# ThinkLib/Sail

Measured on AMD Instinct MI355X. Metric: Msamples/s (paths x bounces) at 1920x1080 Cornell box, higher is better.
Workload: dtype f32; 1 GPU; cornell_box_readme_C2; width=1920, height=1080, bounces=8, spp=1024, launch_spp=1024, partition=tiles64x1, processes=one

## Files before the change

sail_amd/capi.py:

```python
from __future__ import annotations

import ctypes
import os
from typing import Optional, Sequence

import numpy as np

_HERE = os.path.dirname(os.path.abspath(__file__))
LIB_PATH = os.environ.get("SAIL_HIP_LIB") or os.path.join(_HERE, "lib", "libsail_hip.so")

SAIL_OK = 0
FLAG_AOV = 1
FLAG_SEGMENT_COUNT = 2
ACCUM_SUM, ACCUM_MIX, ACCUM_COMPAT8 = 0, 1, 2
PART_TILES, PART_SAMPLES = 0, 1
FILTER_COLOR, FILTER_GAMMA, FILTER_TONEMAPPING, FILTER_WINDOW = 0, 1, 2, 3
FILTER_WAVELET, FILTER_NORMAL, FILTER_POSITION = 4, 5, 6
DEBUG_CULL_MIN_PRIMS, DEBUG_FORCE_GENERIC, DEBUG_CULL_FMA, DEBUG_SAMPLE_GROUPS, DEBUG_FORCE_RCCL = 1, 2, 3, 4, 5
DEBUG_WAVEFRONT = 6
DEBUG_GROUP_ROUNDS = 7
DEBUG_CULL_GROUP_ROUNDS = 8
DEBUG_JIT = 9
DEBUG_JIT_WAIT = 10
DEBUG_JIT_NT = 12
DEBUG_JIT_NS = 11
DEBUG_JIT_VALUES_AFTER = 13
KERNEL_JIT_NONE, KERNEL_JIT_PENDING, KERNEL_JIT_READY, KERNEL_JIT_FAILED = 0, 1, 2, 3
JIT_MODE_FLAT, JIT_MODE_CULL, JIT_MODE_ROOM = 0, 1, 2
DEBUG_DEFAULTS: dict = {}

EXPORTS = (
    "sail_create", "sail_create_multi", "sail_set_debug", "sail_destroy", "sail_last_error", "sail_device_count", "sail_device_info", "sail_set_scene",
    "sail_update_objects", "sail_set_accum_mode", "sail_set_partition", "sail_set_launch_samples",
    "sail_render", "sail_render_schedule", "sail_reset", "sail_sync", "sail_readback", "sail_read_accum",
    "sail_filter", "sail_get_stats", "sail_camera", "sail_jitter_inverse", "sail_schedule",
    "sail_comm_unique_id", "sail_comm_init", "sail_reduce", "sail_accum_device_ptr", "sail_partition_tiles",
    "sail_prim_bounds", "sail_math_probe", "sail_pick", "sail_kernel_name", "sail_filter_ms",
    "sail_abi_version", "sail_accum_parts", "sail_save_accum", "sail_load_accum", "sail_jit_compile",
    "sail_get_kernel_info", "sail_kernel_ready", "sail_set_jit_cache", "sail_jit_prebuild",
    "sail_jit_value_key", "sail_jit_spec_key", "sail_plan_settle", "sail_jit_resident",
    "sail_plan_reduce", "sail_plan_keep", "sail_plan_load_part", "sail_plan_last_bounce",
    "sail_noise_mark", "sail_noise_estimate", "sail_plan_until", "sail_render_until",
    "sail_set_active_tiles", "sail_get_active_tiles", "sail_plan_adaptive", "sail_adaptive_defaults", "sail_render_adaptive",
    "sail_denoise_defaults", "sail_denoise",
    "sail_temporal_defaults", "sail_gbuffer", "sail_temporal_begin", "sail_temporal_resolve", "sail_temporal_read",
    "sail_temporal_load_history",
    "sail_temporal_moments", "sail_temporal_load_moments", "sail_temporal_read_moments",
    "sail_temporal_filter_defaults", "sail_temporal_filter",
    "sail_move_objects", "sail_temporal_pending_motion",
    "sail_albedo", "sail_albedo_load", "sail_albedo_read", "sail_denoise_albedo", "sail_temporal_filter_albedo",
)


class SailError(RuntimeError):
    pass
# ... 970 lines not shown
```

sail_amd/csrc/sail_capi.cpp:

```cpp
#include <hip/hip_runtime.h>
#include <dlfcn.h>
#include <math.h>
#include <algorithm>
#include <cmath>
#include <stdarg.h>
#include <stdio.h>
#include <stdlib.h>
#include <string.h>
#include <string>
#include <vector>
#include "sail_ctx.h"

namespace {

thread_local std::string g_create_error;

float gdiv(float a, float b) { return a * (1.0f / b); }

int texel(float c, int size) {
  if (c != c) return 0;
  const float s = floorf(c * (float)size);
  if (!(s >= 0.0f)) return 0;
  if (s >= (float)(size - 1)) return size - 1;
  return (int)s;
// ... 154 lines not shown
          for (int k = 0; k < 3; k++) {
            volatile float f = kd * sc[q][k];
            f = f * kInvPI;
            if (!std::isfinite((float)f)) matteOk = false;
          }
      }
    }
    if (emPosZero && matteOk) *quietRows |= 1u << i;
    else if (!(matteOk && !emBlack)) skip = false;
  }
  *skipSort = (any && skip) ? 1 : 0;
}
bool valueSpecFor(const SailJitSpec& types, const std::vector<uint32_t>& rowWords, const float* tp, int tn, int jit, SailJitSpec* out) {
  const bool cornellSet = (types.ks & ~SAIL_KSET_CORNELL_SHAPES) == 0 && (types.km & ~SAIL_KSET_CORNELL_MATS) == 0 &&
                          (types.kt & ~SAIL_KSET_CORNELL_TEX) == 0 && types.kl == 0;
  if (!cornellSet || types.mode != SAIL_JIT_MODE_FLAT || types.rows <= 0 || types.tn != 0 || tn < 0 || tn > kSailJitMaxFlatTp ||
      rowWords.size() != (size_t)types.rows * 32 || (tn > 0 && !tp))
    return false;
  *out = types;
  out->rowWords = rowWords;
  out->tpWords.resize((size_t)tn * 16);
  if (tn > 0) memcpy(out->tpWords.data(), tp, sizeof(float) * 16 * (size_t)tn);
  out->rowForm = out->rowShade = out->rowQuiet = 0;
  if ((jit & 32) && types.rows <= kSailJitRowRecordMax) {
    out->rowForm = 1;
    std::vector<SailPrim> prims((size_t)types.rows);
    memcpy(prims.data(), rowWords.data(), sizeof(SailPrim) * prims.size());
    uint32_t quiet = 0;
    int skip = 0;
    lastBounceRows(prims, tp, tn, types.km, false, &quiet, &skip);
    out->rowShade = (int)(quiet & ((1u << types.rows) - 1u));
    out->rowQuiet = out->rowShade;
  }
  return true;
}
void refreshValues(sail_ctx* c) {
  if (!c->subs.empty() || c->valueSlot.have || !c->typesSlot.have || !settledFor(c->settled, c->jitValuesAfter)) return;
  SailJitSpec spec;
  if (!valueSpecFor(c->typesSlot.spec, c->rowWords, c->tpRows.data(), c->tn, c->jit, &spec)) return;
  c->valueSlot.adopt(c->device, c->stream, spec);
}
void refreshJit(sail_ctx* c) {
  if (!c->subs.empty()) return;
  SailJitSpec spec;
  int mode = 0;
  const bool have = jitSpecFor(c, &spec, &mode);
  if (have == c->typesSlot.have && (!have || sailJitSpecEqual(spec, c->typesSlot.spec))) return;
  dropValues(c);
  c->typesTwin.drop(c->device, c->stream);
  if (have) c->typesSlot.adopt(c->device, c->stream, spec);
  else c->typesSlot.drop(c->device, c->stream);
}
JitSlot* maskedTwin(sail_ctx* c, JitSlot& twin, const JitSlot& base) {
  SailJitSpec want = base.spec;
  want.masked = 1;
  if (!twin.have || !sailJitSpecEqual(twin.spec, want)) twin.adopt(c->device, c->stream, want);
  return twin.poll(c->device, c->jitWait) ? &twin : nullptr;
}
JitSlot* runningSlot(sail_ctx* c, bool masked, bool wavefront) {
  if (wavefront) return nullptr;
  if (c->valueSlot.poll(c->device, 0)) {
    JitSlot* s = masked ? maskedTwin(c, c->valueTwin, c->valueSlot) : &c->valueSlot;
    if (s) return s;
  }
  if (c->typesSlot.poll(c->device, c->jitWait)) return masked ? maskedTwin(c, c->typesTwin, c->typesSlot) : &c->typesSlot;
  return nullptr;
// ... 657 lines not shown
  if (!c) return SAIL_E_INVALID;
  if (option == SAIL_DEBUG_FORCE_RCCL) {
    if (c->subs.empty() || c->groupLocal)
      return fail(c, SAIL_E_INVALID, "SAIL_DEBUG_FORCE_RCCL needs a multi-device context of distinct devices");
    for (sail_ctx* s : c->subs) if (int rc = flushQueued(s)) return relay(c, rc, s);
    const int nd = (int)c->subs.size();
    if (value && c->groupComms.empty()) {
      if (!g_rccl.load()) return fail(c, SAIL_E_RCCL, "librccl not loadable");
      std::vector<int> dev((size_t)nd);
      for (int i = 0; i < nd; i++) dev[i] = c->subs[i]->device;
      c->groupComms.assign((size_t)nd, nullptr);
      const int r = g_rccl.commInitAll(c->groupComms.data(), nd, dev.data());
      if (r) {
        c->groupComms.clear();
        return fail(c, SAIL_E_RCCL, "ncclCommInitAll: %s", g_rccl.errStr ? g_rccl.errStr(r) : "?");
      }
    } else if (!value && nd == 1 && !c->groupComms.empty()) {
      for (sail_ctx* s : c->subs) { (void)hipSetDevice(s->device); (void)hipStreamSynchronize(s->stream); }
      for (nccl_comm_t cm : c->groupComms) if (cm) g_rccl.commDestroy(cm);
      c->groupComms.clear();
    }
    c->dirty = true;
    return SAIL_OK;
  }
  for (sail_ctx* s : c->subs) if (int rc = sail_set_debug(s, option, value)) return relay(c, rc, s);
  if (int rc = flushQueued(c)) return rc;
  switch (option) {
    case SAIL_DEBUG_CULL_MIN_PRIMS: c->cullMinPrims = value; break;
    case SAIL_DEBUG_FORCE_GENERIC: c->forceGeneric = value; break;
    case SAIL_DEBUG_CULL_FMA: c->cullFma = value; break;
    case SAIL_DEBUG_SAMPLE_GROUPS: c->forceGroups = value; break;
    case SAIL_DEBUG_WAVEFRONT: c->wavefront = value; break;
    case SAIL_DEBUG_JIT:
      if ((c->jit ^ value) & 32) { const uint64_t s = c->settled; dropValues(c); c->settled = s; }
      c->jit = value;
      break;
    case SAIL_DEBUG_JIT_NT:
      if (value != 0 && value != 128 && value != 256 && value != 512 && value != 1024)
        return fail(c, SAIL_E_INVALID, "sail_set_debug: threads per workgroup must be 0 (default), 128, 256, 512 or 1024");
      c->jitNt = value;
      break;
    case SAIL_DEBUG_JIT_NS:
      if (value != 0 && value != 1 && value != 4 && value != 16)
        return fail(c, SAIL_E_INVALID, "sail_set_debug: samples in flight must be 0 (default), 1, 4 or 16");
      c->jitNs = value;
      break;
    case SAIL_DEBUG_JIT_WAIT:
      if (value < -1) return fail(c, SAIL_E_INVALID, "sail_set_debug: jit wait must be >= -1");
      c->jitWait = value;
      break;
    case SAIL_DEBUG_JIT_VALUES_AFTER:
      c->jitValuesAfter = value;
      if (value < 0) { const uint64_t s = c->settled; dropValues(c); c->settled = s; }
      break;
    case SAIL_DEBUG_GROUP_ROUNDS:
      if (value <= 0) return fail(c, SAIL_E_INVALID, "sail_set_debug: group rounds must be > 0");
      c->flatGroupRounds = value;
      break;
    case SAIL_DEBUG_CULL_GROUP_ROUNDS:
      if (value <= 0) return fail(c, SAIL_E_INVALID, "sail_set_debug: group rounds must be > 0");
      c->cullGroupRounds = value;
      break;
    default: return fail(c, SAIL_E_INVALID, "sail_set_debug: unknown option %d", option);
  }
  refreshJit(c);
  refreshValues(c);
  return SAIL_OK;
// ... 614 lines not shown
```

sail_amd/csrc/sail_geom.h:

```cpp
#pragma once
#if !defined(__HIPCC_RTC__)
#include <hip/hip_runtime.h>
#include <stdint.h>
#endif
#include "sail_device.h"
#include "sail_math.h"

using namespace sm;

#define D __device__ __forceinline__

namespace {

constexpr float kMaxDistance = 1e5f, kEps = 1e-5f, kOneMinusEps = 0.9999f, kInf = 1e5f;
constexpr float kPI = 3.141592653589793f, kInvPI = 0.3183098861837907f;
constexpr float kPiOver2 = 1.570796326794896f, kPiOver4 = 0.785398163397448f;

struct V3 { float x, y, z; };
struct V2 { float x, y; };
D V3 v3(float x, float y, float z) { V3 r; r.x = x; r.y = y; r.z = z; return r; }
D V3 v3s(float s) { return v3(s, s, s); }
D V2 v2(float x, float y) { V2 r; r.x = x; r.y = y; return r; }
D V3 operator+(V3 a, V3 b) { return v3(a.x + b.x, a.y + b.y, a.z + b.z); }
D V3 operator-(V3 a, V3 b) { return v3(a.x - b.x, a.y - b.y, a.z - b.z); }
// ... 13 lines not shown
D V3 vmin(V3 a, V3 b) { return v3(fmin_(a.x, b.x), fmin_(a.y, b.y), fmin_(a.z, b.z)); }
D V3 vmax(V3 a, V3 b) { return v3(fmax_(a.x, b.x), fmax_(a.y, b.y), fmax_(a.z, b.z)); }
D V3 vclamp01(V3 x) { return v3(clamp_(x.x, 0.0f, 1.0f), clamp_(x.y, 0.0f, 1.0f), clamp_(x.z, 0.0f, 1.0f)); }
D bool isBlack(V3 a) { return a.x == 0.0f && a.y == 0.0f && a.z == 0.0f; }
D V3 reflect_(V3 I, V3 N) { return I - (2.0f * dot(N, I)) * N; }
D V3 refract_(V3 I, V3 N, float eta) {
  const float dni = dot(N, I);
  const float k = 1.0f - eta * eta * (1.0f - dni * dni);
  if (k < 0.0f) return v3s(0.0f);
  return eta * I - (eta * dni + sqrtf_(k)) * N;
}
D V3 worldToLocal(V3 v, V3 ns, V3 ss, V3 ts) { return v3(dot(v, ss), dot(v, ts), dot(v, ns)); }
D V3 localToWorld(V3 v, V3 ns, V3 ss, V3 ts) {
  return v3(ss.x * v.x + ts.x * v.y + ns.x * v.z, ss.y * v.x + ts.y * v.y + ns.y * v.z,
            ss.z * v.x + ts.z * v.y + ns.z * v.z);
}
D float dotX(V3 a, V3 b) { return fma_(a.z, b.z, fma_(a.y, b.y, a.x * b.x)); }
D V3 crossX(V3 a, V3 b) {
  return v3(fma_(a.y, b.z, -(a.z * b.y)), fma_(a.z, b.x, -(a.x * b.z)), fma_(a.x, b.y, -(a.y * b.x)));
}
D V3 localToWorldX(V3 v, V3 ns, V3 ss, V3 ts) {
  return v3(fma_(ns.x, v.z, fma_(ts.x, v.y, ss.x * v.x)), fma_(ns.y, v.z, fma_(ts.y, v.y, ss.y * v.x)),
            fma_(ns.z, v.z, fma_(ts.z, v.y, ss.z * v.x)));
}
D V3 W2L(V3 v) {
  return v3(fma_(v.y, 0.0f, v.x * 0.0f) - v.z, fma_(v.z, 0.0f, fma_(v.y, 0.0f, v.x)), fma_(v.z, 0.0f, fma_(v.x, 0.0f, v.y)));
}
D V3 L2W(V3 v) {
  return v3(fma_(v.z, 0.0f, fma_(v.x, 0.0f, v.y)), fma_(v.y, 0.0f, v.x * 0.0f) + v.z, fma_(v.z, 0.0f, fma_(v.y, 0.0f, -v.x)));
}
D bool equalZero(float x) { return x < 1e-3f && x > -1e-3f; }
D float sgn(int rev) { return rev ? -1.0f : 1.0f; }

D bool quadratic(float A, float B, float C, float& t0, float& t1) {
  const float discrim = B * B - 4.0f * A * C;
  if (discrim < 0.0f) return false;
  const float rootDiscrim = sqrtf_(discrim);
  float q;
  if (B < 0.0f) q = -0.5f * (B - rootDiscrim);
  else q = -0.5f * (B + rootDiscrim);
  t0 = fdiv(q, A);
  t1 = fdiv(C, q);
  if (t0 > t1) { const float tmp = t0; t0 = t1; t1 = tmp; }
  return true;
}

struct Ray { V3 o, d; float rx, ry, rz; };
D Ray mkRay(V3 o, V3 d) {
  Ray r; r.o = o; r.d = d;
  const float mx = fmaxf(fmaxf(fabsf(d.x), fabsf(d.y)), fabsf(d.z)), mn = fminf(fminf(fabsf(d.x), fabsf(d.y)), fabsf(d.z));
  if (__builtin_expect(__builtin_amdgcn_ballot_w64(!(mn >= 0x1p-126f && mx <= 0x1p126f)) == 0ull, 1)) {
    const float y0 = __builtin_amdgcn_rcpf(d.x), y1 = __builtin_amdgcn_rcpf(d.y), y2 = __builtin_amdgcn_rcpf(d.z);
    r.rx = fma_(fma_(-d.x, y0, 1.0f), y0, y0);
    r.ry = fma_(fma_(-d.y, y1, 1.0f), y1, y1);
    r.rz = fma_(fma_(-d.z, y2, 1.0f), y2, y2);
  } else {
    r.rx = 1.0f / d.x; r.ry = 1.0f / d.y; r.rz = 1.0f / d.z;
  }
  return r;
}
struct Hit {
  float d; V3 hit, normal, dpdu, dpdv; bool into; int matRow; V3 sc, emission; int matCategory;
  float nd;
  bool axis;
};
struct Ctx {
  const float* tp; const float* lt; const int32_t* lightObjRow; const SailPrim* prims;
  const SailPrim* cprims;
  const float* tpl;
  bool rowCopy, tpCopy;
  const unsigned long long* typeMasks;
  int n, tn, ln;
  uint32_t matMask, texMask, lightMask;
  float fcx, fcy;
  int shadowAnyHit;
  int cullPrims;
  int cullFma;
  int cullPrimary;
  uint32_t kShapes, kMats, kTex, kLights;
};
#define HAS(set, id) (((set) >> (id)) & 1u)

template <typename T> using ConstAS = const __attribute__((address_space(4))) T;
template <typename T> D const T& constRow(const T* base, int i) { return *(const T*)((ConstAS<T>*)base + i); }
#if defined(SAIL_JIT) && defined(SAIL_JIT_ROWVALS) && SAIL_JIT_ROWVALS && SAIL_JIT_N > 0
#define SAIL_ROWVALS 1
template <class... T> constexpr int wordCount(T...) { return (int)sizeof...(T); }
static_assert(sizeof(SailPrim) == 128, "a row is 32 words");
static_assert(wordCount(SAIL_JIT_ROW_WORDS) == SAIL_JIT_N * 32, "32 words per row");
constexpr int kTpC = SAIL_JIT_TPN;
static_assert(wordCount(SAIL_JIT_TP_WORDS) == (kTpC > 0 ? kTpC * 16 : 1), "16 words per texParams row");
struct PrimWordsC { uint32_t w[SAIL_JIT_N * 32]; };
struct PrimTabC { SailPrim r[SAIL_JIT_N]; };
struct TpWordsC { uint32_t w[kTpC > 0 ? kTpC * 16 : 1]; };
struct TpTabC { float v[kTpC > 0 ? kTpC * 16 : 1]; };
constexpr PrimWordsC kPrimW = {{SAIL_JIT_ROW_WORDS}};
constexpr TpWordsC kTpW = {{SAIL_JIT_TP_WORDS}};
constexpr PrimTabC kPrimTab = __builtin_bit_cast(PrimTabC, kPrimW);
constexpr TpTabC kTpTab = __builtin_bit_cast(TpTabC, kTpW);
#define PRIM(c, i) (kPrimTab.r[(i)])
#else
#define SAIL_ROWVALS 0
#define PRIM(c, i) constRow<SailPrim>((c).prims, (i))
#endif
#if SAIL_ROWVALS && defined(SAIL_JIT_ROWSHADE) && SAIL_JIT_ROWSHADE
#define SAIL_ROWSHADE 1
#else
#define SAIL_ROWSHADE 0
#endif

D V3 P3(const SailPrim& p, int k) { return v3(p.a[k], p.a[k + 1], p.a[k + 2]); }
D float TP(const Ctx& c, int row, int col) {
#if SAIL_ROWVALS
  return kTpTab.v[row * 16 + col];
#else
  if (c.tpCopy) return c.tpl[row * 16 + col];
  return constRow<float>(c.tp, row * 16 + col);
#endif
}
D V3 TP3(const Ctx& c, int row, int col) { return v3(TP(c, row, col), TP(c, row, col + 1), TP(c, row, col + 2)); }

D int matCat(const SailPrim& p) { return (int)(short)(p.cats & 0xffff); }
D int texCat(const SailPrim& p) { return p.cats >> 16; }
D bool needsUV(const SailPrim& p) { return texCat(p) != SAIL_TEX_UNIFORM; }
D V3 getSurfaceColor(const Ctx& c, V2 uv, const SailPrim& p) {
  const int texRow = p.texRow, cat = texCat(p);
  if (cat == SAIL_TEX_UNIFORM) return TP3(c, texRow, 1);
  if (cat < 0 || cat >= 32 || !((c.texMask >> cat) & 1u)) return v3s(0.0f);
  if (c.cullPrims &&
      ((cat == SAIL_TEX_CHECKERBOARD && HAS(c.kTex, SAIL_TEX_CHECKERBOARD)) ||
       (cat == SAIL_TEX_CHECKERBOARD2 && HAS(c.kTex, SAIL_TEX_CHECKERBOARD2)))) {
    const bool cb1 = cat == SAIL_TEX_CHECKERBOARD;
    const float size = cb1 ? TP(c, texRow, 1) : TP(c, texRow, 7);
    const float sx = fdiv(uv.x, size), sy = fdiv(uv.y, size);
    const float qx = floorf(sx), qy = floorf(sy);
    if (cb1) {
      const float width = fdiv(0.5f * TP(c, texRow, 2), size);
      const float fx = sx - qx, fy = sy - qy;
      const bool in_outline = (fx < width || fx > 1.0f - width) || (fy < width || fy > 1.0f - width);
      return in_outline ? v3s(0.5f) : v3s(1.0f);
    }
    return (to_int(qx + qy) % 2 == 0) ? TP3(c, texRow, 1) : TP3(c, texRow, 4);
// ... 103 lines not shown
  if (x.x < mn.x + 0.0001f) h.sc = v3(0.25f, 0.75f, 0.25f);
  else if (x.x > mx.x - 0.0001f) h.sc = v3(0.25f, 0.25f, 0.75f);
  else if (x.y < mn.y + 0.0001f) h.sc = v3s(1.0f);
  else if (x.y > mx.y - 0.0001f) h.sc = v3s(1.0f);
  else if (x.z > mn.z + 0.0001f) h.sc = v3s(1.0f);
  else h.sc = v3s(0.0f);
}

D void boxHit(const Ctx& c, const SailPrim& p, const Ray& r, float t, Hit& h, bool cornell) {
  h.hit = r.o + t * r.d;
  const float s = cornell ? -1.0f : sgn(p.rev);
  h.normal = s * normalForCornellbox(r.o + t * r.d, p);
  dpdBox(h.normal, h.dpdu, h.dpdv);
  const V3 mn = P3(p, 0), mx = P3(p, 3), x = h.hit;
  if (cornell) {
    if (x.x < mn.x + 0.0001f) h.sc = v3(0.25f, 0.75f, 0.25f);
    else if (x.x > mx.x - 0.0001f) h.sc = v3(0.25f, 0.25f, 0.75f);
    else if (x.y < mn.y + 0.0001f) h.sc = v3s(1.0f);
    else if (x.y > mx.y - 0.0001f) h.sc = v3s(1.0f);
    else if (x.z > mn.z + 0.0001f) h.sc = v3s(1.0f);
    else h.sc = v3s(0.0f);
  } else {
    V2 uv = v2(0.0f, 0.0f);
    if (needsUV(p)) {
      const V3 tr = mx - mn, hh = h.hit - mn;
      if (hh.x < mn.x + 0.0001f || hh.x > mx.x - 0.0001f) uv = v2(fdiv(hh.y, tr.y), fdiv(hh.z, tr.z));
      else if (hh.y < mn.y + 0.0001f || hh.y > mx.y - 0.0001f) uv = v2(fdiv(hh.x, tr.x), fdiv(hh.z, tr.z));
      else uv = v2(fdiv(hh.x, tr.x), fdiv(hh.y, tr.y));
    }
    h.sc = getSurfaceColor(c, uv, p);
  }
}

D float sphereT(const SailPrim& p, const Ray& r0, V3* hitOut) {
  const V3 c = P3(p, 0);
  const float rad = p.a[3];
  const V3 d = W2L(r0.d), o = W2L(r0.o - c);
  const float a = dot(d, d), b = 2.0f * dot(o, d), cc = dot(o, o) - rad * rad;
  float t1 = 0.0f, t2 = 0.0f;
  if (!quadratic(a, b, cc, t1, t2)) return kMaxDistance;
  if (t2 < kEps) return kMaxDistance;
  float t = t1;
  if (t1 < kEps) t = t2;
  if (t >= kMaxDistance) return kMaxDistance;
  if (!testBoundbox(r0, c - v3s(rad), c + v3s(rad))) return kMaxDistance;
  if (hitOut) *hitOut = o + t * d;
  return t;
}
D float phiOf(float y, float x) {
  float phi = atan2f_(y, x);
  if (phi < 0.0f) phi += 2.0f * kPI;
  return phi;
}
D V3 dpduRot(V3 hit) { return v3(-2.0f * kPI * hit.y, 2.0f * kPI * hit.x, 0.0f); }
D V3 crossZa(V3 a, V3 b) {
  return v3(fma_(b.y, -0.0f, a.y * b.z), fma_(b.x, 0.0f, -(a.x * b.z)), a.x * b.y - a.y * b.x);
}
D V3 crossZb(V3 a, V3 b) {
  return v3(fma_(a.y, 0.0f, -(a.z * b.y)), fma_(a.x, -0.0f, a.z * b.x), a.x * b.y - a.y * b.x);
}
D void sphereHit(const Ctx& c, const SailPrim& p, V3 hl, Hit& h) {
  const float rad = p.a[3];
  const float theta = acosf_(clamp_(fdiv(hl.z, rad), -1.0f, 1.0f));
  V2 uv = v2(0.0f, 0.0f);
  if (needsUV(p)) {
    V3 hit = hl;
    if (hit.x == 0.0f && hit.y == 0.0f) hit.x = 1e-5f * rad;
    uv = v2(fdiv(phiOf(hit.y, hit.x), 2.0f * kPI), fdiv(theta, kPI));
  }
  const float th2 = theta;
  const float zRadius = sqrtf_(hl.x * hl.x + hl.y * hl.y);
  const float invZRadius = rcp_rn(zRadius);
  const float cosPhi = hl.x * invZRadius, sinPhi = hl.y * invZRadius;
  const V3 dpdu = dpduRot(hl);
  const V3 dpdv = kPI * v3(hl.z * cosPhi, hl.z * sinPhi, -rad * sinf_(th2));
  const V3 nl = normalize(crossZb(dpdv, dpdu));
  h.sc = getSurfaceColor(c, uv, p);
  h.hit = L2W(hl) + P3(p, 0);
  h.normal = L2W(nl);
  h.dpdu = L2W(dpdu);
// ... 514 lines not shown
      best = t;
      if (c.shadowAnyHit && best > kEps && best < kOneMinusEps) break;
    }
  }
  return best;
}

struct Sweep { float best; int bi; V3 bhl; };
D Sweep sweepRay(const Ctx& c, const Ray& r, bool primary) {
  float best = kMaxDistance;
  int bi = -1;
  V3 bhl = v3s(0.0f);
  const bool cull = c.cullPrims && (!primary || c.cullPrimary);
  if (cull) {
    candSweep<true>(c, r, kMaxDistance, best, bi, bhl);
    Sweep sw; sw.best = best; sw.bi = bi; sw.bhl = bhl;
    return sw;
  }
  if constexpr (kRows > 0) {
    if (!c.cullPrims) {
      sweepRows<0>(c, r, best, bi, bhl);
      Sweep sw; sw.best = best; sw.bi = bi; sw.bhl = bhl;
      return sw;
    }
  }
  for (int i = 0; i < c.n; i++) {
    V3 hl = v3s(0.0f);
    const float t = primT(c, PRIM(c, i), r, &hl);
    if (t < best) { best = t; bi = i; bhl = hl; }
  }
  Sweep sw; sw.best = best; sw.bi = bi; sw.bhl = bhl;
  return sw;
}
D V3 quadLocalHit(const SailPrim& p, const Ray& r, float t) {
  const V3 d = W2L(r.d), o = W2L(r.o - P3(p, 0));
  return o + t * d;
}
D V3 rectLocalHit(const SailPrim& p, const Ray& r, float t) {
  const RectFrame f = rectFrame(p);
  const V3 d = worldToLocal(r.d, f.normal, f.ss, f.ts);
  const V3 o = worldToLocal(r.o - P3(p, 0), f.normal, f.ss, f.ts);
  return o + t * d;
}
template <bool RECOMP_HL = false, bool BOXU = false>
D Hit hitRecord(const Ctx& c, const Ray& r, const Sweep& sw) {
  const float best = sw.best;
  const int bi = sw.bi;
  Hit h;
  h.d = best;
  const SailPrim& p = c.rowCopy ? c.cprims[bi] : PRIM(c, bi);
#define BHL (RECOMP_HL ? quadLocalHit(p, r, best) : sw.bhl)
  constexpr bool boxU = BOXU;
  const bool localU = c.cullPrims != 0;
  const uint32_t kLocal = c.kShapes & ((1u << SAIL_SPHERE) | (1u << SAIL_CONE) | (1u << SAIL_CYLINDER) |
                                       (1u << SAIL_HYPERBOLOID) | (1u << SAIL_PARABOLOID) | (1u << SAIL_DISK));
  if (boxU && ((HAS(c.kShapes, SAIL_CUBE) && p.type == SAIL_CUBE) ||
               (HAS(c.kShapes, SAIL_CORNELLBOX) && p.type == SAIL_CORNELLBOX))) {
    boxHit(c, p, r, best, h, HAS(c.kShapes, SAIL_CORNELLBOX) && p.type == SAIL_CORNELLBOX);
  } else if (localU && ((kLocal >> p.type) & 1u)) {
    localHit(c, p, BHL, h);
  } else
  switch (p.type) {
    case SAIL_CUBE: if (!boxU && HAS(c.kShapes, SAIL_CUBE)) { cubeHit(c, p, r, best, h); break; } __builtin_unreachable();
    case SAIL_SPHERE: if (!localU && HAS(c.kShapes, SAIL_SPHERE)) { sphereHit(c, p, BHL, h); break; } __builtin_unreachable();
    case SAIL_RECTANGLE: if (HAS(c.kShapes, SAIL_RECTANGLE)) { rectHit(c, p, RECOMP_HL ? rectLocalHit(p, r, best) : sw.bhl, h); break; } __builtin_unreachable();
    case SAIL_CONE: if (!localU && HAS(c.kShapes, SAIL_CONE)) { coneHit(c, p, BHL, h); break; } __builtin_unreachable();
// ... 85 lines not shown
```

sail_amd/csrc/sail_jit.cpp:

```cpp
#include <ctype.h>
#include <dirent.h>
#include <dlfcn.h>
#include <pthread.h>
#include <errno.h>
#include <hip/hip_runtime.h>
#include <hip/hip_version.h>
#include <hip/hiprtc.h>
#include <stdint.h>
#include <stdio.h>
#include <stdlib.h>
#include <string.h>
#include <sys/stat.h>
#include <unistd.h>
#include <algorithm>
#include <chrono>
#include <condition_variable>
#include <map>
#include <memory>
#include <mutex>
#include <string>
#include <thread>
#include <tuple>
#include <vector>

#include "sail_jit.h"

extern const char* const sail_jit_src_names[];
extern const char* const sail_jit_src_texts[];
extern const int sail_jit_src_count;
extern const int sail_trace_phase_timing;

int sailJitThreads(const SailJitSpec& s) { return s.nt ? s.nt : (s.mode == 1 ? 1024 : 256); }
bool sailJitSpecEqual(const SailJitSpec& a, const SailJitSpec& b) {
  const auto t = [](const SailJitSpec& x) {
    return std::tie(x.ks, x.km, x.kt, x.kl, x.mode, x.waves, x.rows, x.ldsFit, x.tn, x.ns, x.nt, x.types[0], x.types[1], x.types[2],
                    x.types[3], x.types[4], x.types[5], x.types[6], x.types[7], x.rowWords, x.tpWords, x.rowForm, x.rowShade, x.rowQuiet, x.masked);
  };
  return t(a) == t(b);
}

namespace {

bool isValue(const SailJitSpec& s) { return !s.rowWords.empty(); }

struct Key {
  SailJitSpec s;
  bool operator<(const Key& o) const {
    const auto t = [](const SailJitSpec& x) {
      return std::tie(x.ks, x.km, x.kt, x.kl, x.mode, x.waves, x.rows, x.ldsFit, x.tn, x.ns, x.nt, x.types[0], x.types[1], x.types[2],
                      x.types[3], x.types[4], x.types[5], x.types[6], x.types[7], x.rowWords, x.tpWords, x.rowForm, x.rowShade, x.rowQuiet, x.masked);
    };
    return t(s) < t(o.s);
  }
};

uint64_t fnv(const void* p, size_t n, uint64_t h = 14695981039346656037ull) {
  const unsigned char* b = static_cast<const unsigned char*>(p);
  for (size_t i = 0; i < n; i++) { h ^= b[i]; h *= 1099511628211ull; }
  return h;
}
uint64_t fnvStr(const std::string& s, uint64_t h) { return fnv(s.data(), s.size() + 1, h); }
std::string hex16(uint64_t v) {
  char b[17];
  snprintf(b, sizeof b, "%016llx", (unsigned long long)v);
  return b;
}

uint64_t sourceHash() {
  static const uint64_t h = [] {
    uint64_t x = fnv("sail-jit-src", 12);
    for (int i = 0; i < sail_jit_src_count; i++) { x = fnvStr(sail_jit_src_names[i], x); x = fnvStr(sail_jit_src_texts[i], x); }
    return x;
  }();
  return h;
}

const char* const kOpts[] = {"-O3", "-std=c++17", "-ffp-contract=off", "-fno-fast-math", "-mllvm", "-vectorize-slp=false"};

std::string defsFor(const SailJitSpec& sp) {
  std::string types;
  for (int i = 0; i < sp.rows; i++) types += (i ? ", " : "") + std::to_string(sp.types[i]);
  std::string vals;
  if (!sp.rowWords.empty()) {
    const auto list = [](const std::vector<uint32_t>& w) {
      std::string s;
      char b[16];
      for (size_t i = 0; i < w.size(); i++) { snprintf(b, sizeof b, i ? ", 0x%08xu" : "0x%08xu", w[i]); s += b; }
      return s.empty() ? std::string("0u") : s;
    };
    vals = (sp.rowForm ? "#define SAIL_JIT_ROWSHADE " + std::to_string(sp.rowShade) + "\n#define SAIL_JIT_ROWQUIET " +
                             std::to_string(sp.rowQuiet) + "\n"
                       : std::string()) + "#define SAIL_JIT_ROWVALS 1\n#define SAIL_JIT_TPN " + std::to_string(sp.tpWords.size() / 16) +
           "\n#define SAIL_JIT_ROW_WORDS " + list(sp.rowWords) + "\n#define SAIL_JIT_TP_WORDS " + list(sp.tpWords) + "\n";
  }
  char defs[768];
  snprintf(defs, sizeof defs,
           "#define SAIL_JIT 1\n#define SAIL_JIT_WAVES %d\n#define SAIL_JIT_CULL %d\n#define SAIL_JIT_FAM %d\n"
           "#define SAIL_JIT_KS 0x%xu\n#define SAIL_JIT_KM 0x%xu\n#define SAIL_JIT_KT 0x%xu\n#define SAIL_JIT_KL 0x%xu\n"
           "#define SAIL_JIT_NT %d\n#define SAIL_JIT_N %d\n#define SAIL_JIT_TYPES %s\n#define SAIL_JIT_LDSFIT %d\n"
           "#define SAIL_JIT_TN %d\n#define SAIL_JIT_NS %d\n#include \"sail_trace.hip\"\n",
           sp.waves, sp.mode == 1, sp.mode == 2, sp.ks, sp.km, sp.kt, sp.kl, sailJitThreads(sp), sp.rows,
           sp.rows ? types.c_str() : "0", sp.ldsFit, sp.tn, sp.ns);
  return (sail_trace_phase_timing ? std::string("#define SAIL_PHASE_TIMING 1\n") : std::string()) +
         (sp.masked ? std::string("#define SAIL_JIT_MASKED 1\n") : std::string()) + vals + defs;
}

struct Rtc {
  decltype(&hiprtcCreateProgram) create;
  decltype(&hiprtcCompileProgram) compile;
  decltype(&hiprtcGetProgramLogSize) logSize;
  decltype(&hiprtcGetProgramLog) log;
  decltype(&hiprtcGetCodeSize) codeSize;
  decltype(&hiprtcGetCode) code;
  decltype(&hiprtcDestroyProgram) destroy;
  decltype(&hiprtcGetErrorString) errStr;
  decltype(&hiprtcVersion) version;
  int major = 0, minor = 0;
};

void waitInFlight();

const Rtc* rtc(std::string& err) {
  static Rtc r;
  static std::string why;
  static std::once_flag once;
// ... 143 lines not shown
  for (const char* o : kOpts) opts.push_back(o);
  r = R.compile(prog, (int)opts.size(), opts.data());
  if (r != HIPRTC_SUCCESS) {
    size_t n = 0;
    R.logSize(prog, &n);
    std::string log(n, '\0');
    if (n) R.log(prog, &log[0]);
    err = std::string(R.errStr(r)) + ": " + log.substr(0, 2000);
    R.destroy(&prog);
    return -1;
  }
  size_t n = 0;
  R.codeSize(prog, &n);
  code.resize(n);
  R.code(prog, code.data());
  R.destroy(&prog);
  if (!n) { err = "hipRTC returned an empty code object"; return -1; }
  return 0;
}

bool validSpec(const SailJitSpec& sp, std::string* err) {
  bool ok = sp.mode >= 0 && sp.mode <= 2 && sp.waves >= 1 && sp.waves <= 8 && sp.rows >= 0 && sp.rows <= kSailJitMaxRows &&
            !(sp.mode == 1 && sp.rows) &&
            (sp.ldsFit == 0 || (sp.ldsFit == 1 && sp.mode == 1)) &&
            (sp.tn == 0 || (sp.tn >= 1 && sp.tn <= kSailJitMaxFlatTp && sp.mode != 1 && sp.rows > 0)) &&
            (sp.ns == 1 || sp.ns == 4 || sp.ns == 16) &&
            (sp.nt == 0 || sp.nt == 128 || sp.nt == 256 || sp.nt == 512 || sp.nt == 1024) && sailJitThreads(sp) / sp.ns >= 16;
  for (int i = 0; ok && i < sp.rows; i++) ok = sp.types[i] >= 1 && sp.types[i] <= 9 && ((sp.ks >> sp.types[i]) & 1u);
  if (ok && (isValue(sp) || !sp.tpWords.empty())) {
    ok = sp.mode == 0 && sp.rows > 0 && sp.tn == 0 && sp.rowWords.size() == (size_t)sp.rows * 32 &&
         sp.tpWords.size() % 16 == 0 && sp.tpWords.size() <= (size_t)kSailJitMaxFlatTp * 16;
    for (int i = 0; ok && i < sp.rows; i++) ok = sp.rowWords[(size_t)i * 32] == (uint32_t)sp.types[i];
  }
  if (!ok) *err = "invalid kernel specialisation";
  return ok;
}

struct Entry {
  std::mutex m;
  std::condition_variable cv;
  int state = 0;
  std::vector<char> code;
  std::string err;
  uint64_t id = 0;
  double compileMs = 0.0;
  int fromCache = 0;
  bool pinned = false;
};
std::mutex g_mapMutex;
std::map<std::pair<std::string, Key>, std::shared_ptr<Entry>> g_code;
std::map<std::pair<std::string, Key>, int> g_holds;

uint64_t codeId(const std::vector<char>& code) {
  const unsigned char* b = reinterpret_cast<const unsigned char*>(code.data());
  const size_t n = code.size();
  auto u16 = [&](size_t o) { return o + 2 <= n ? (uint64_t)b[o] | (uint64_t)b[o + 1] << 8 : 0; };
  auto u32 = [&](size_t o) { return o + 4 <= n ? u16(o) | u16(o + 2) << 16 : 0; };
  auto u64 = [&](size_t o) { return o + 8 <= n ? u32(o) | u32(o + 4) << 32 : 0; };
  if (n < 64 || memcmp(b, "\177ELF", 4) != 0 || b[4] != 2) return fnv(code.data(), n);
  const uint64_t shoff = u64(0x28), shentsize = u16(0x3a), shnum = u16(0x3c), shstrndx = u16(0x3e);
  if (shentsize < 64 || shstrndx >= shnum || shoff + shnum * shentsize > n) return fnv(code.data(), n);
  const uint64_t strOff = u64(shoff + shstrndx * shentsize + 0x18), strSize = u64(shoff + shstrndx * shentsize + 0x20);
  if (strOff + strSize > n) return fnv(code.data(), n);
  uint64_t h = fnv("sail-code", 9);
  for (uint64_t k = 0; k < shnum; k++) {
    const size_t e = shoff + k * shentsize;
// ... 376 lines not shown
```

sail_amd/csrc/sail_jit.h:

```cpp
#pragma once
#include <hip/hip_runtime.h>
#include <stdint.h>
#include <string>
#include <vector>

constexpr int kSailJitMaxRows = 8;
constexpr int kSailJitMaxFlatTp = 32;
constexpr int kSailJitRowRecordMax = 3;
struct SailJitSpec {
  uint32_t ks = 0, km = 0, kt = 0, kl = 0;
  int mode = 0;
  int waves = 6;
  int rows = 0;
  int ldsFit = 0;
  int tn = 0;
  int ns = 1;
  int nt = 0;
  int types[kSailJitMaxRows] = {};
  std::vector<uint32_t> rowWords, tpWords;
  int rowForm = 0, rowShade = 0, rowQuiet = 0;
  int masked = 0;
};
bool sailJitSpecEqual(const SailJitSpec& a, const SailJitSpec& b);
int sailJitThreads(const SailJitSpec& s);

struct SailJitKernel {
  hipFunction_t plain = nullptr, grouped = nullptr;
  uint64_t buildId = 0;
  double compileMs = 0.0;
  int fromCache = 0;
};
int sail_jit_kernels(int device, const SailJitSpec& spec, int wait_ms, SailJitKernel* out, std::string* err);
void sail_jit_hold(int device, const SailJitSpec& spec, int delta);
int sail_jit_code(const char* arch, const SailJitSpec& spec, void* code, size_t* bytes, std::string* err);
void sail_jit_set_cache_dir(const char* dir);
constexpr int kSailJitMaxValueObjects = 32;
int sail_jit_code_to_dir(const char* arch, const SailJitSpec& spec, const char* dir, std::string* err);
uint64_t sail_precompiled_build_id(const char* kernel);
int sail_jit_key(const char* arch, const SailJitSpec& spec, uint64_t* key, std::string* defs, std::string* err);
void sail_jit_resident_values(int* code_objects, int* modules);
```

sail_amd/csrc/sail_trace.hip:

```cpp
#ifndef SAIL_TRACE_HIP
#define SAIL_TRACE_HIP
#if !defined(__HIPCC_RTC__)
#include <hip/hip_runtime.h>
#include <stdint.h>
#endif
#include "sail_device.h"
#include "sail_geom.h"
#include "sail_scan.h"
#include "sail_shade.h"


#if defined(SAIL_PHASE_TIMING) && SAIL_PHASE_TIMING
extern "C" __device__ unsigned long long g_sailPhase[12];
__device__ unsigned long long g_sailPhase[12];
#endif

namespace {

struct TileWork { int ownedTile, sub, kBeg, kEnd, bid; };
template <bool MASKED>
D int ownedTileIndex(const SailTraceArgs& A, int ownedTile) {
  if constexpr (MASKED) return A.tileMap[ownedTile];
  else return A.rank + ownedTile * A.world;
}
// ... 161 lines not shown
    if (pixLane) sAcc[li] = acc;
  }
  const float s = ((float)x + 0.5f) / (float)A.W, t = ((float)y + 0.5f) / (float)A.H;
  const bool tri0 = s + t <= 1.0f;
  const V3 eye = v3(A.eye[0], A.eye[1], A.eye[2]);
  unsigned segs = 0;
  unsigned long long segsW = 0;
  PhaseClock pc;
#if SAIL_PHASE_TIMING
  for (int q = 0; q < 12; q++) pc.acc[q] = 0;
  pc.t = __builtin_amdgcn_s_memtime();
#endif
  for (int k = tw.kBeg; k < tw.kEnd; k += NS) {
    const int ks = k + mySlot;
    const bool inRange = NS == 1 || ks < tw.kEnd;
    const SailSample& S = constRow<SailSample>(A.samples, NS == 1 ? k : (inRange ? ks : k));
    const bool aovs = A.aovN || A.aovP;
    bool alive = valid && inRange;
    int pixel = li;
    auto pathSeed = [&](int h) { if constexpr (NS == 1) return S.seed; else return sSeed[h / kPX]; };
    Ray ray;
    {
      const V3 d0 = v3(S.d[0][0], S.d[0][1], S.d[0][2]), d1 = v3(S.d[1][0], S.d[1][1], S.d[1][2]);
      const V3 d2 = v3(S.d[2][0], S.d[2][1], S.d[2][2]), d3 = v3(S.d[3][0], S.d[3][1], S.d[3][2]);
      ray = mkRay(eye, tri0 ? (d0 + (d2 - d0) * s + (d1 - d0) * t) : (d3 + (d1 - d3) * (1.0f - s) + (d2 - d3) * (1.0f - t)));
    }
    V3 fpdf = v3s(1.0f);
    E_STORE(li, v3s(0.0f));
    for (int depth = 1; depth <= A.maxBounces; depth++) {
      Sweep sw;
      sw.best = kMaxDistance; sw.bi = -1; sw.bhl = v3s(0.0f);
      int key = 0;
      if constexpr (CULL) segsW += (unsigned long long)__popcll(__builtin_amdgcn_ballot_w64(alive));
      if (alive) {
        if constexpr (!CULL) segs++;
        sw = sweepRay(c, ray, depth == 1);
        if (sw.best >= kMaxDistance) {
          if (depth == 1 && aovs && k + pixel / kPX == A.spp - 1) {
            const size_t g = (size_t)homeY(pixel) * A.W + homeX(pixel);
            const V3 qn = v3s(0.0f) / 2.0f + 0.5f, qp = normalize(v3s(0.0f));
            if (A.aovN) A.aovN[g] = make_float4(qn.x, qn.y, qn.z, 1.0f);
            if (A.aovP) A.aovP[g] = make_float4(qp.x, qp.y, qp.z, 1.0f);
          }
          alive = false;
        } else if (byPrim) {
          key = 1 + sw.bi;
          if constexpr (FAM && !CULL && kCornellRow >= 0) {
            if (sw.bi == kCornellRow) {
              const SailPrim& cp = PRIM(c, kCornellRow);
              const V3 h = ray.o + sw.best * ray.d, mn = P3(cp, 0), mx = P3(cp, 3);
              const int face = h.x < mn.x + 0.0001f ? 0 : h.x > mx.x - 0.0001f ? 1 : h.y < mn.y + 0.0001f ? 2
                             : h.y > mx.y - 0.0001f ? 3 : h.z < mn.z + 0.0001f ? 4 : 5;
              key = 1 + kRows + face;
            }
          }
        } else {
          const SailPrim& p = PRIM(c, sw.bi);
          int mc = matCat(p);
          mc = (mc >= 0 && mc < 5) ? mc : 0;
          key = 1 + mc * 10 + p.type;
        }
      }
      const bool lastB = !CULL && !FAM && depth == A.maxBounces;
      if constexpr (!CULL && !FAM) {
        if (lastB) __builtin_amdgcn_s_setprio(0);
        if (lastB && alive && ((A.lastQuietRows >> (sw.bi & 31)) & 1u) != 0u &&
            !(depth == 1 && aovs && k + pixel / kPX == A.spp - 1)) {
          E_STORE(pixel, E_LOAD(pixel) + v3s(0.0f) * fpdf);
          alive = false;
// ... 72 lines not shown
      if (alive) {
        if (!sortNow) {
          keyG = key;
        } else if constexpr (kPack == 2) {
          const float4 q0 = sSt4[0][li], q1 = sSt4[1][li], q2 = sSt4[2][li];
          const int pk = __float_as_int(q2.z);
          keyG = __float_as_int(q2.w);
          ray.o = v3(q0.x, q0.y, q0.z);
          ray.d = v3(q0.w, q1.x, q1.y);
          fpdf = v3(q1.z, q1.w, q2.x);
          sw.best = q2.y;
          pixel = pk & 1023;
          sw.bi = pk >> 10;
          sw.bhl = v3s(0.0f);
        } else {
          const float2 q0 = sSt2[0][li], q1 = sSt2[1][li], q2 = sSt2[2][li], q3 = sSt2[3][li], q4 = sSt2[4][li];
          const int pk = __float_as_int(sSt2[5][li].x);
          keyG = __float_as_int(sSt2[5][li].y);
          ray.o = v3(q0.x, q0.y, q1.x);
          ray.d = v3(q1.y, q2.x, q2.y);
          fpdf = v3(q3.x, q3.y, q4.x);
          sw.best = q4.y;
          pixel = pk & 1023;
          sw.bi = pk >> 10;
          sw.bhl = v3s(0.0f);
        }
        ray.rx = ray.ry = ray.rz = 0.0f;
        {
          const int k0 = __builtin_amdgcn_readfirstlane(keyG);
          const bool mixedW = __builtin_amdgcn_ballot_w64(keyG != k0) != 0ull;
          if (mixedW) __builtin_amdgcn_s_setprio(kPrioMixed);
          else __builtin_amdgcn_s_setprio(0);
        }
        c.fcx = (float)homeX(pixel) + 0.5f;
        c.fcy = (float)homeY(pixel) + 0.5f;
        const float seed = pathSeed(pixel) + (float)depth;
#define SAIL_BOUNCE_REST(ins, Q)                                                                   \
        PHASE_MARK(pc, 1);                                                                         \
        if (depth == 1 && aovs && k + pixel / kPX == A.spp - 1) {                                  \
          const size_t g = (size_t)homeY(pixel) * A.W + homeX(pixel);                              \
          const V3 qn = ins.normal / 2.0f + 0.5f, qp = normalize(ins.hit);                         \
          if (A.aovN) A.aovN[g] = make_float4(qn.x, qn.y, qn.z, 1.0f);                             \
          if (A.aovP) A.aovP[g] = make_float4(qp.x, qp.y, qp.z, 1.0f);                             \
        }                                                                                          \
        V3 e = (Q) ? v3s(0.0f) : E_LOAD(pixel);         \
        if (!(!CULL && depth == A.maxBounces && shadeLast(c, ins, seed, fpdf, e))) {               \
          if constexpr (kShCompact) {                                                              \
            shadeBounceP(c, ins, ray, seed, fpdf, e, pc, sp);             \
            eLit = sp.eLit;                                                                        \
          } else {                                                                                 \
            shadeBounce(c, ins, ray, seed, fpdf, e, pc);                                           \
          }                                                                                        \
        }                                                                                          \
        if constexpr (!(Q)) E_STORE(pixel, e);
#if SAIL_ROWSHADE
        bounceU<true, FAM && !CULL>(c, ray, sw,
                                    [&](const Hit& ins, auto quiet) __attribute__((always_inline)) {
          SAIL_BOUNCE_REST(ins, decltype(quiet)::value)
        });
#else
        const Hit ins = hitRecordU<true, FAM && !CULL>(c, ray, sw);
        SAIL_BOUNCE_REST(ins, false)
#endif
#undef SAIL_BOUNCE_REST
      }
      if constexpr (kShCompact) {
        if (c.ln > 0) {
          const bool pend = alive && sp.pending;
          __syncthreads();
          const unsigned long long bm = __builtin_amdgcn_ballot_w64(pend);
          if (bm != 0ull) {
            int base = 0;
            if (lane == 0) base = atomicAdd(&sShCnt[shph], __popcll(bm));
            base = __shfl(base, 0, 64);
            if (pend) {
              const int d = base + (int)__builtin_amdgcn_mbcnt_hi((unsigned)(bm >> 32),
                                                                  __builtin_amdgcn_mbcnt_lo((unsigned)bm, 0u));
              const V3 o = sp.hit, dl = sp.toLight;
              if constexpr (kPack == 2) {
                sSt4[0][d] = make_float4(o.x, o.y, o.z, dl.x);
                sSt4[1][d] = make_float4(dl.y, dl.z, eLit.x, eLit.y);
                sSt4[2][d] = make_float4(eLit.z, __int_as_float(pixel), 0.0f, 0.0f);
              } else {
                sSt2[0][d] = make_float2(o.x, o.y); sSt2[1][d] = make_float2(o.z, dl.x);
                sSt2[2][d] = make_float2(dl.y, dl.z); sSt2[3][d] = make_float2(eLit.x, eLit.y);
                sSt2[4][d] = make_float2(eLit.z, __int_as_float(pixel));
              }
            }
          }
          __syncthreads();
          const int nSh = sShCnt[shph];
          if (li == 0) sShCnt[shph ^ 1] = 0;
          shph ^= 1;
          if (li < nSh) {
            V3 o, dl, el;
            int pix;
            if constexpr (kPack == 2) {
// ... 76 lines not shown
```

Measured before the change: 116,000 Msamples/s.

## Defer sphere-row intersection into the key-sorted phase to cut divergence

Splits the sphere quadratic into a discriminant test and a root solve. On middle bounces in the flat JIT value kernel, the full sphere solve is deferred: rays that pass the cheap test and may hit the sphere are given a sort key for the sphere row, and the solve runs only after key-based regrouping, so whole waves resolve it together. Deferred rays that then miss everything are killed. This aims to reduce divergent sqrt/div work inside the sweep, at the cost of an extra key class, a second transform of the ray, and extra control flow. It is on by default, with a new JIT flag bit to disable it.

```diff
diff --git a/sail_amd/capi.py b/sail_amd/capi.py
--- a/sail_amd/capi.py
+++ b/sail_amd/capi.py
@@ -21,6 +21,7 @@
 DEBUG_GROUP_ROUNDS = 7
 DEBUG_CULL_GROUP_ROUNDS = 8
 DEBUG_JIT = 9
+JIT_NO_ROWDEFER = 64
 DEBUG_JIT_WAIT = 10
 DEBUG_JIT_NT = 12
 DEBUG_JIT_NS = 11
diff --git a/sail_amd/csrc/sail_capi.cpp b/sail_amd/csrc/sail_capi.cpp
--- a/sail_amd/csrc/sail_capi.cpp
+++ b/sail_amd/csrc/sail_capi.cpp
@@ -210,6 +210,10 @@
     out->rowShade = (int)(quiet & ((1u << types.rows) - 1u));
     out->rowQuiet = out->rowShade;
   }
+  out->rowDefer = -1;
+  if (!(jit & 64))
+    for (int i = types.rows - 1; i >= 0; i--)
+      if (types.types[i] == SAIL_SPHERE) out->rowDefer = i;
   return true;
 }
 void refreshValues(sail_ctx* c) {
@@ -933,7 +937,7 @@
     case SAIL_DEBUG_SAMPLE_GROUPS: c->forceGroups = value; break;
     case SAIL_DEBUG_WAVEFRONT: c->wavefront = value; break;
     case SAIL_DEBUG_JIT:
-      if ((c->jit ^ value) & 32) { const uint64_t s = c->settled; dropValues(c); c->settled = s; }
+      if ((c->jit ^ value) & (32 | 64)) { const uint64_t s = c->settled; dropValues(c); c->settled = s; }
       c->jit = value;
       break;
     case SAIL_DEBUG_JIT_NT:
diff --git a/sail_amd/csrc/sail_geom.h b/sail_amd/csrc/sail_geom.h
--- a/sail_amd/csrc/sail_geom.h
+++ b/sail_amd/csrc/sail_geom.h
@@ -69,17 +69,26 @@
 D bool equalZero(float x) { return x < 1e-3f && x > -1e-3f; }
 D float sgn(int rev) { return rev ? -1.0f : 1.0f; }
 
+template <int PART>
+D bool quadratic(float A, float B, float C, float& t0, float& t1, float& discrim) {
+  if constexpr (PART != 2) {
+    discrim = B * B - 4.0f * A * C;
+    if (discrim < 0.0f) return false;
+  }
+  if constexpr (PART != 1) {
+    const float rootDiscrim = sqrtf_(discrim);
+    float q;
+    if (B < 0.0f) q = -0.5f * (B - rootDiscrim);
+    else q = -0.5f * (B + rootDiscrim);
+    t0 = fdiv(q, A);
+    t1 = fdiv(C, q);
+    if (t0 > t1) { const float tmp = t0; t0 = t1; t1 = tmp; }
+  }
+  return true;
+}
 D bool quadratic(float A, float B, float C, float& t0, float& t1) {
-  const float discrim = B * B - 4.0f * A * C;
-  if (discrim < 0.0f) return false;
-  const float rootDiscrim = sqrtf_(discrim);
-  float q;
-  if (B < 0.0f) q = -0.5f * (B - rootDiscrim);
-  else q = -0.5f * (B + rootDiscrim);
-  t0 = fdiv(q, A);
-  t1 = fdiv(C, q);
-  if (t0 > t1) { const float tmp = t0; t0 = t1; t1 = tmp; }
-  return true;
+  float discrim = 0.0f;
+  return quadratic<0>(A, B, C, t0, t1, discrim);
 }
 
 struct Ray { V3 o, d; float rx, ry, rz; };
@@ -145,6 +154,15 @@
 #else
 #define SAIL_ROWSHADE 0
 #endif
+#if defined(SAIL_JIT_ROWDEFER) && SAIL_JIT_ROWDEFER >= 0
+#define SAIL_ROWDEFER 1
+static_assert(SAIL_ROWVALS, "a deferred row: in a value kernel");
+static_assert(!SAIL_JIT_CULL && !SAIL_JIT_FAM, "a deferred row: in the flat form");
+constexpr int kDeferRow = SAIL_JIT_ROWDEFER;
+#else
+#define SAIL_ROWDEFER 0
+constexpr int kDeferRow = -1;
+#endif
 
 D V3 P3(const SailPrim& p, int k) { return v3(p.a[k], p.a[k + 1], p.a[k + 2]); }
 D float TP(const Ctx& c, int row, int col) {
@@ -314,20 +332,30 @@
   }
 }
 
-D float sphereT(const SailPrim& p, const Ray& r0, V3* hitOut) {
+struct SphereQuad { V3 o, d; float a, b, cc, discrim; };
+template <int PART>
+D float sphereT(const SailPrim& p, const Ray& r0, V3* hitOut, SphereQuad& q) {
   const V3 c = P3(p, 0);
   const float rad = p.a[3];
-  const V3 d = W2L(r0.d), o = W2L(r0.o - c);
-  const float a = dot(d, d), b = 2.0f * dot(o, d), cc = dot(o, o) - rad * rad;
   float t1 = 0.0f, t2 = 0.0f;
-  if (!quadratic(a, b, cc, t1, t2)) return kMaxDistance;
+  if constexpr (PART != 2) {
+    q.d = W2L(r0.d); q.o = W2L(r0.o - c);
+    q.a = dot(q.d, q.d); q.b = 2.0f * dot(q.o, q.d); q.cc = dot(q.o, q.o) - rad * rad;
+    if (!quadratic<1>(q.a, q.b, q.cc, t1, t2, q.discrim)) return kMaxDistance;
+  }
+  if constexpr (PART == 1) return 0.0f;
+  quadratic<2>(q.a, q.b, q.cc, t1, t2, q.discrim);
   if (t2 < kEps) return kMaxDistance;
   float t = t1;
   if (t1 < kEps) t = t2;
   if (t >= kMaxDistance) return kMaxDistance;
   if (!testBoundbox(r0, c - v3s(rad), c + v3s(rad))) return kMaxDistance;
-  if (hitOut) *hitOut = o + t * d;
+  if (hitOut) *hitOut = q.o + t * q.d;
   return t;
+}
+D float sphereT(const SailPrim& p, const Ray& r0, V3* hitOut) {
+  SphereQuad q;
+  return sphereT<0>(p, r0, hitOut, q);
 }
 D float phiOf(float y, float x) {
   float phi = atan2f_(y, x);
@@ -908,6 +936,45 @@
   Sweep sw; sw.best = best; sw.bi = bi; sw.bhl = bhl;
   return sw;
 }
+#if SAIL_ROWDEFER
+static_assert(kDeferRow < kRows && kRowType[kDeferRow] == SAIL_SPHERE && HAS(SAIL_JIT_KS, SAIL_SPHERE),
+              "the deferred row is a Sphere the kernel intersects");
+template <int I>
+D void sweepRowsDefer(const Ctx& c, const Ray& r, bool defer, float& best, int& bi, V3& bhl, bool& cand) {
+  if constexpr (I < kRows) {
+    if constexpr (I == kDeferRow) {
+      SphereQuad q;
+      const bool live = sphereT<1>(PRIM(c, I), r, nullptr, q) < kMaxDistance;
+      if (defer) {
+        cand = live && !(q.b > 0.0f && q.cc > 0.0f);
+      } else if (live) {
+        V3 hl = v3s(0.0f);
+        const float t = sphereT<2>(PRIM(c, I), r, &hl, q);
+        if (t < best) { best = t; bi = I; bhl = hl; }
+      }
+    } else {
+      V3 hl = v3s(0.0f);
+      const float t = primTy(c, kRowType[I], PRIM(c, I), r, &hl);
+      if (t < best) { best = t; bi = I; bhl = hl; }
+    }
+    sweepRowsDefer<I + 1>(c, r, defer, best, bi, bhl, cand);
+  }
+}
+D Sweep sweepRayDefer(const Ctx& c, const Ray& r, bool defer, bool& cand) {
+  Sweep sw;
+  sw.best = kMaxDistance; sw.bi = -1; sw.bhl = v3s(0.0f);
+  cand = false;
+  sweepRowsDefer<0>(c, r, defer, sw.best, sw.bi, sw.bhl, cand);
+  return sw;
+}
+D void sphereResolve(const Ctx& c, const Ray& r, Sweep& sw) {
+  const SailPrim& p = PRIM(c, kDeferRow);
+  const Ray rr = mkRay(r.o, r.d);
+  SphereQuad q;
+  const float t = sphereT<0>(p, rr, nullptr, q);
+  if (t < sw.best || (t == sw.best && kDeferRow < sw.bi)) { sw.best = t; sw.bi = kDeferRow; }
+}
+#endif
 D V3 quadLocalHit(const SailPrim& p, const Ray& r, float t) {
   const V3 d = W2L(r.d), o = W2L(r.o - P3(p, 0));
   return o + t * d;
diff --git a/sail_amd/csrc/sail_jit.cpp b/sail_amd/csrc/sail_jit.cpp
--- a/sail_amd/csrc/sail_jit.cpp
+++ b/sail_amd/csrc/sail_jit.cpp
@@ -34,7 +34,7 @@
 bool sailJitSpecEqual(const SailJitSpec& a, const SailJitSpec& b) {
   const auto t = [](const SailJitSpec& x) {
     return std::tie(x.ks, x.km, x.kt, x.kl, x.mode, x.waves, x.rows, x.ldsFit, x.tn, x.ns, x.nt, x.types[0], x.types[1], x.types[2],
-                    x.types[3], x.types[4], x.types[5], x.types[6], x.types[7], x.rowWords, x.tpWords, x.rowForm, x.rowShade, x.rowQuiet, x.masked);
+                    x.types[3], x.types[4], x.types[5], x.types[6], x.types[7], x.rowWords, x.tpWords, x.rowForm, x.rowShade, x.rowQuiet, x.rowDefer, x.masked);
   };
   return t(a) == t(b);
 }
@@ -48,7 +48,7 @@
   bool operator<(const Key& o) const {
     const auto t = [](const SailJitSpec& x) {
       return std::tie(x.ks, x.km, x.kt, x.kl, x.mode, x.waves, x.rows, x.ldsFit, x.tn, x.ns, x.nt, x.types[0], x.types[1], x.types[2],
-                      x.types[3], x.types[4], x.types[5], x.types[6], x.types[7], x.rowWords, x.tpWords, x.rowForm, x.rowShade, x.rowQuiet, x.masked);
+                      x.types[3], x.types[4], x.types[5], x.types[6], x.types[7], x.rowWords, x.tpWords, x.rowForm, x.rowShade, x.rowQuiet, x.rowDefer, x.masked);
     };
     return t(s) < t(o.s);
   }
@@ -90,7 +90,9 @@
     };
     vals = (sp.rowForm ? "#define SAIL_JIT_ROWSHADE " + std::to_string(sp.rowShade) + "\n#define SAIL_JIT_ROWQUIET " +
                              std::to_string(sp.rowQuiet) + "\n"
-                       : std::string()) + "#define SAIL_JIT_ROWVALS 1\n#define SAIL_JIT_TPN " + std::to_string(sp.tpWords.size() / 16) +
+                       : std::string()) +
+           (sp.rowDefer >= 0 ? "#define SAIL_JIT_ROWDEFER " + std::to_string(sp.rowDefer) + "\n" : std::string()) +
+           "#define SAIL_JIT_ROWVALS 1\n#define SAIL_JIT_TPN " + std::to_string(sp.tpWords.size() / 16) +
            "\n#define SAIL_JIT_ROW_WORDS " + list(sp.rowWords) + "\n#define SAIL_JIT_TP_WORDS " + list(sp.tpWords) + "\n";
   }
   char defs[768];
@@ -300,6 +302,7 @@
          sp.tpWords.size() % 16 == 0 && sp.tpWords.size() <= (size_t)kSailJitMaxFlatTp * 16;
     for (int i = 0; ok && i < sp.rows; i++) ok = sp.rowWords[(size_t)i * 32] == (uint32_t)sp.types[i];
   }
+  if (ok && sp.rowDefer != -1) ok = isValue(sp) && sp.rowDefer >= 0 && sp.rowDefer < sp.rows && sp.types[sp.rowDefer] == 2;
   if (!ok) *err = "invalid kernel specialisation";
   return ok;
 }
diff --git a/sail_amd/csrc/sail_jit.h b/sail_amd/csrc/sail_jit.h
--- a/sail_amd/csrc/sail_jit.h
+++ b/sail_amd/csrc/sail_jit.h
@@ -19,6 +19,7 @@
   int types[kSailJitMaxRows] = {};
   std::vector<uint32_t> rowWords, tpWords;
   int rowForm = 0, rowShade = 0, rowQuiet = 0;
+  int rowDefer = -1;
   int masked = 0;
 };
 bool sailJitSpecEqual(const SailJitSpec& a, const SailJitSpec& b);
diff --git a/sail_amd/csrc/sail_trace.hip b/sail_amd/csrc/sail_trace.hip
--- a/sail_amd/csrc/sail_trace.hip
+++ b/sail_amd/csrc/sail_trace.hip
@@ -217,9 +217,23 @@
       sw.best = kMaxDistance; sw.bi = -1; sw.bhl = v3s(0.0f);
       int key = 0;
       if constexpr (CULL) segsW += (unsigned long long)__popcll(__builtin_amdgcn_ballot_w64(alive));
+#if SAIL_ROWDEFER
+      static_assert(!CULL && !FAM && kRows < kKeys, "a deferred row: in the flat form, sorted by winning row");
+      const bool deferB = depth > 1 && depth < A.maxBounces;
+      bool cand = false;
+#endif
       if (alive) {
         if constexpr (!CULL) segs++;
+#if SAIL_ROWDEFER
+        sw = sweepRayDefer(c, ray, deferB, cand);
+#else
         sw = sweepRay(c, ray, depth == 1);
+#endif
+#if SAIL_ROWDEFER
+        if (cand) {
+          key = 1 + kDeferRow;
+        } else
+#endif
         if (sw.best >= kMaxDistance) {
           if (depth == 1 && aovs && k + pixel / kPX == A.spp - 1) {
             const size_t g = (size_t)homeY(pixel) * A.W + homeX(pixel);
@@ -358,6 +372,15 @@
           if (mixedW) __builtin_amdgcn_s_setprio(kPrioMixed);
           else __builtin_amdgcn_s_setprio(0);
         }
+#if SAIL_ROWDEFER
+        if (deferB) {
+          PHASE_MARK(pc, 1);
+          if (keyG == 1 + kDeferRow) sphereResolve(c, ray, sw);
+          if (sw.best >= kMaxDistance) alive = false;
+          PHASE_MARK(pc, 0);
+        }
+#endif
+        if (alive) {
         c.fcx = (float)homeX(pixel) + 0.5f;
         c.fcy = (float)homeY(pixel) + 0.5f;
         const float seed = pathSeed(pixel) + (float)depth;
@@ -389,6 +412,7 @@
         SAIL_BOUNCE_REST(ins, false)
 #endif
 #undef SAIL_BOUNCE_REST
+        }
       }
       if constexpr (kShCompact) {
         if (c.ln > 0) {
```

Result: faster. 118,300 Msamples/s (median of 6 runs) (+2.0%).
